# pymc-devs/pymc

Hardware: AMD Instinct MI355X
Metric: effective samples/sec (and leapfrog steps/sec), 10k-param hierarchical logistic regression, one NUTS chain per GPU (higher is better)
Workload: dtype f64

## Files before the change

pymc_amd/csrc/engine.hip:

```cpp
#include <hip/hip_runtime.h>

#include <algorithm>
#include <atomic>
#include <chrono>
#include <cmath>
#include <cstdio>
#include <cstdlib>
#include <cstring>
#include <mutex>
#include <thread>
#include <utility>
#include <ctime>
#include <string>
#include <vector>

#include "kernels.h"
#include "small_kernel.h"
#include "mixture_kernel.h"
#include "loglik_kernel.h"
#include "predictive_kernel.h"
#include "nuts_mi355.h"
#include "pcg64_stream.h"
#include "advi.h"

// ... 53 lines not shown
  int cap = 0, used = 0;
  int64_t ring_full = 0;
  void reset() { side = 0; n = 0; cap = 0; used = 0; }
  template <class F>
  void begin(int d, int dir, int last, F dir_of) {
    cap = 0; used = 0;
    for (int e = d + 1; e <= last; ++e)
      if (dir_of(e) == -dir) { cap = std::min(1 << std::min(e, 30), ring); break; }
  }
  int leaf(int dir, int* slot, int* k) {
    if (n > 0 && side == dir) { *slot = (int)(head % (unsigned)ring); *k = used++; ++head; --n; return EP_REPLAY; }
    if (cap > 0 && n < cap) { side = -dir; *k = n; *slot = (int)((head + (unsigned)n) % (unsigned)ring); ++n; return EP_PAIRED; }
    if (cap > 0 && n >= ring) ++ring_full;
    *slot = -1; *k = -1;
    return EP_PLAIN;
  }
};
extern "C" int64_t nuts_edge_pair_plan(const int32_t* dirs, int32_t n_dirs, int32_t n_doublings, int32_t spec, int32_t max_depth,
                                       int32_t ring, int32_t* out, int64_t out_cap) {
  if (!dirs || !out || n_doublings < 0 || n_doublings > n_dirs || n_doublings > 20 || ring < 1) { g_err = "nuts_edge_pair_plan: bad argument"; return -1; }
  EdgePlan ep;
  ep.ring = ring;
  int64_t n = 0;
  const int last = std::min(std::min(spec, max_depth - 1), n_dirs - 1);
  for (int d = 0; d < n_doublings; ++d) {
    ep.begin(d, dirs[d], last, [&](int e) { return (int)dirs[e]; });
    for (int j = 0; j < (1 << d); ++j, ++n) {
      int slot, k;
      const int kind = ep.leaf(dirs[d], &slot, &k);
      if (n >= out_cap) { g_err = "nuts_edge_pair_plan: output too small"; return -1; }
      int32_t* o = out + 5 * n;
      o[0] = d; o[1] = j; o[2] = kind; o[3] = slot; o[4] = k;
    }
  }
  return n;
}

#define PROF_RUN_MIN 16
#define SMALL_MAX_ELEMS 16384
#define SMALL_MAX_N 1024

struct nuts_model {
  ModelDev md{};
  hipStream_t stream = nullptr;
  std::vector<void*> owned;
  double* q_dev = nullptr;
  double* g_dev = nullptr;
  double* lp_dev = nullptr;
  double* host_pin = nullptr;
  std::vector<nuts_data_ref> data_refs;
  int64_t data_epoch = 0;
  double* set_pin = nullptr; int64_t set_pin_len = 0; hipEvent_t set_ev = nullptr;
  int rows_grid = 0, mvn_grid = 0, ept = 1;
  bool has_prog = false;
  int rows_rpl = 2, rows_alternate = 1, rows_flip = 0, rows_occ = 4;
  int vector_one_xcd = 0;
  int ga_struct_ok = 0;
  int ga_par = 0;
  int64_t dom_units = 0;
  int explicit_pre = 0;
  int64_t alg_bytes = 0;
  bool profile = false;
  std::vector<hipEvent_t> ev;
  std::vector<int32_t> ev_units;
  int run_open = 0;
  int64_t runs_seen = 0;
  size_t ev_used = 0;
  int64_t dom_launches = 0;
  int sample_every = 1;
  hipStream_t own_stream = nullptr;
  struct nuts_group* group = nullptr;
  bool g_active = false;
  int gslot = 0;
  int n_chains = 0;
  int64_t pool_extra = 0;
  int64_t orphan_elems = 0, factor_elems = 0;
  double rows_pack_s = 0.0;
  int64_t rows_xt_len = 0, rows_y_len = 0;
  int ep_ok = 0, ep_par = 0;
  double *ep_ring = nullptr, *ep_part = nullptr, *ep_bpart = nullptr, *ep_def_loc = nullptr;
  int64_t ep_ring_bytes = 0, ep_shadows = 0, ep_replays = 0;
  int64_t ep_dropped = 0;
  int64_t ep_ring_full = 0;
  int ep_turns = 0;
  struct EpLaunch {
    int kind = EP_PLAIN, slot = 0, sj = 0, sfold = 0, first = 0;
    EvalIO sio{}; ArenaDev sA{};
  } ep_launch;
  std::vector<LinDev> lins_host;
  std::vector<nuts_factor> fac_host;
  double *ll_q = nullptr, *ll_stage = nullptr, *ll_par = nullptr, *ll_sc = nullptr, *ll_lfact = nullptr;
  int32_t* ll_dead = nullptr;
  int64_t ll_stage_n = 0, ll_par_n = 0;
  int n_waic = 0;

  template <typename T>
  T* keep(T* p) {
    owned.push_back((void*)p);
    return p;
  }
};

extern "C" int nuts_device_count(void) {
  int n = 0;
  if (hipGetDeviceCount(&n) != hipSuccess) return 0;
  return n;
}
extern "C" int nuts_set_device(int device) {
  HIPCHK(hipSetDevice(device));
  return NUTS_OK;
}
extern "C" const char* nuts_last_error(void) { return g_err.c_str(); }

#define GRP_MAXC MFM_MAXC
struct nuts_group {
  std::mutex mu;
  hipStream_t stream = nullptr;
  nuts_model* member[GRP_MAXC] = {};
  int n = 0;
  int nactive = 0, npend = 0;
  std::atomic<unsigned> gen{0};
  MvaLeafArgs pend[GRP_MAXC];
  int64_t launches[GRP_MAXC + 1] = {};
  int cap = MVM_MAXC;
  ModelDev* md_dev = nullptr;
  const nuts_model* md_of = nullptr;
  double* dpack = nullptr;
  MfmChainConst* konst_dev = nullptr;
  MfmChainConst konst_host[GRP_MAXC] = {};
  bool konst_set[GRP_MAXC] = {};
  int kind = 0;
  GaLeafArgs gpend[GAL_MAXC];
  int rows_flip = 0;
  GalConst* gal_konst_dev = nullptr;
  GalConst gal_konst_host[GAL_MAXC] = {};
  bool gal_konst_set[GAL_MAXC] = {};
  int rows_lds = 1;
};
static_assert(GAM_MAXNC == MVM_MAXC && GAL_MAXC == GAM_MAXC && GAL_MAXC <= GRP_MAXC, "group sizes");

static nuts_model* group_base(nuts_group* g) {
  for (int i = 0; i < GRP_MAXC; ++i) if (g->member[i]) return g->member[i];
  return nullptr;
}

template <typename Leaf, int N>
static void group_order(const Leaf* pend, int nc, int (&order)[N]) {
  for (int a = 0; a < N; ++a) order[a] = a;
  for (int a = 1; a < nc; ++a)
    for (int b = a; b > 0 && pend[order[b]].slot < pend[order[b - 1]].slot; --b) std::swap(order[b], order[b - 1]);
}

static void group_submitted(nuts_group* g, int nc) {
  g->launches[nc]++;
  g->npend = 0;
  g->gen.fetch_add(1, std::memory_order_release);
}

static GalConst gal_const(const GaLeafArgs& L) {
  GalConst k{};
  k.A = L.A; k.A.uniforms = nullptr; k.A.log_uniforms = nullptr; k.Emax = L.Emax; k.st = L.st;
  k.ga_part = L.ga_part; k.ga_bpart = L.ga_bpart; k.ga_ticket = L.ga_ticket; k.def_loc = L.def_loc; k.max_depth = L.max_depth; k.slot = L.slot;
  return k;
}

static void group_flush_rows_locked(nuts_group* g);
// ... 1602 lines not shown
extern "C" int nuts_model_set_data(nuts_model* m, int32_t data_id, const double* values, int64_t n) {
  if (!m || !values) { g_err = "null argument"; return NUTS_E_ARG; }
  if (data_id < 0 || data_id >= (int)m->data_refs.size()) { g_err = "nuts_model_set_data: no such data vector"; return NUTS_E_ARG; }
  const nuts_data_ref& r = m->data_refs[data_id];
  if (n != r.size) { g_err = "nuts_model_set_data: the length of a data vector cannot change"; return NUTS_E_ARG; }
  HIPCHK(hipStreamSynchronize(m->stream));
  HIPCHK(hipMemcpy(const_cast<double*>(m->md.pool) + r.offset, values, (size_t)n * sizeof(double), hipMemcpyHostToDevice));
  m->data_epoch++;
  return NUTS_OK;
}

extern "C" int nuts_model_set_data_many(nuts_model* m, int32_t count, const int32_t* data_ids, const double* values, const int64_t* lens) {
  if (!m || count < 0 || (count > 0 && (!data_ids || !values || !lens))) { g_err = "null argument"; return NUTS_E_ARG; }
  int64_t total = 0;
  for (int i = 0; i < count; ++i) {
    if (data_ids[i] < 0 || data_ids[i] >= (int)m->data_refs.size()) { g_err = "nuts_model_set_data_many: no such data vector"; return NUTS_E_ARG; }
    if (lens[i] != m->data_refs[data_ids[i]].size) { g_err = "nuts_model_set_data_many: the length of a data vector cannot change"; return NUTS_E_ARG; }
    total += lens[i];
  }
  if (total == 0) return NUTS_OK;
  if (m->set_pin_len < total) {
    if (m->set_ev) HIPCHK(hipEventSynchronize(m->set_ev));
    if (m->set_pin) hipHostFree(m->set_pin);
    m->set_pin = nullptr; m->set_pin_len = 0;
    HIPCHK(hipHostMalloc((void**)&m->set_pin, (size_t)total * sizeof(double), hipHostMallocDefault));
    m->set_pin_len = total;
  }
  if (!m->set_ev) HIPCHK(hipEventCreateWithFlags(&m->set_ev, hipEventDisableTiming));
  else HIPCHK(hipEventSynchronize(m->set_ev));
  std::memcpy(m->set_pin, values, (size_t)total * sizeof(double));
  int64_t at = 0;
  for (int i = 0; i < count;) {
    const int64_t off0 = m->data_refs[data_ids[i]].offset;
    int64_t run = lens[i];
    int j = i + 1;
    while (j < count && m->data_refs[data_ids[j]].offset == off0 + run) { run += lens[j]; ++j; }
    if (run > 0)
      HIPCHK(hipMemcpyAsync(const_cast<double*>(m->md.pool) + off0, m->set_pin + at, (size_t)run * sizeof(double), hipMemcpyHostToDevice, m->stream));
    at += run;
    i = j;
  }
  HIPCHK(hipEventRecord(m->set_ev, m->stream));
  m->data_epoch++;
  return NUTS_OK;
}

static void group_remove_model(struct nuts_group* g, nuts_model* m);
extern "C" void nuts_model_destroy(nuts_model* m) {
  if (!m) return;
  if (m->stream) hipStreamSynchronize(m->stream);
  if (m->set_ev) hipEventDestroy(m->set_ev);
  if (m->set_pin) hipHostFree(m->set_pin);
  if (m->group) group_remove_model(m->group, m);
  for (void* p : m->owned) if (p) hipFree(p);
  for (void* p : {(void*)m->ll_q, (void*)m->ll_stage, (void*)m->ll_par, (void*)m->ll_sc, (void*)m->ll_dead, (void*)m->ll_lfact}) if (p) hipFree(p);
  for (auto e : m->ev) hipEventDestroy(e);
  if (m->host_pin) hipHostFree(m->host_pin);
  if (m->own_stream) hipStreamDestroy(m->own_stream);
  delete m;
}

extern "C" int nuts_model_debug_ticks(nuts_model* m, int64_t* out) {
  if (!m || !out) return NUTS_E_ARG;
  HIPCHK(hipStreamSynchronize(m->stream));
  HIPCHK(hipMemcpy(out, m->md.ticks, 64 * sizeof(long long), hipMemcpyDeviceToHost));
  return NUTS_OK;
}

extern "C" int32_t nuts_model_ndim(const nuts_model* m) { return m ? m->md.n : -1; }
extern "C" int nuts_model_get_scalar(const nuts_model* m, const char* name, double* out) {
  if (!m || !name || !out) return NUTS_E_ARG;
  const std::string k(name);
  if (k == "rows_group_aligned") *out = m->md.lg.ga;
  else if (k == "rows_group_block") *out = m->md.lg.ga_gpw;
  else if (k == "rows_packed") *out = m->md.lg.ga ? m->md.lg.ga_pack : 0;
  else if (k == "rows_pack_build_s") *out = m->rows_pack_s;
  else if (k == "edge_pair") *out = m->ep_ok;
  else if (k == "edge_pair_ring_bytes") *out = (double)m->ep_ring_bytes;
  else if (k == "edge_pair_shadows") *out = (double)m->ep_shadows;
  else if (k == "edge_pair_replays") *out = (double)m->ep_replays;
  else if (k == "edge_pair_turns") *out = m->ep_turns;
  else if (k == "edge_pair_dropped") *out = (double)m->ep_dropped;
  else if (k == "edge_pair_ring_full") *out = (double)m->ep_ring_full;
  else if (k == "rows_aux_workgroups") *out = m->md.lg.ga ? m->md.lg.ga_naux : 0;
  else if (k == "mixture_workgroups") *out = m->md.has_mix ? m->md.mix.nwg : 0;
  else if (k == "glm_workgroups") *out = m->md.has_glm ? m->md.glm.nwg : 0;
  else if (k == "glm_row_stride") *out = m->md.has_glm ? m->md.glm.xstride : 0;
  else if (k == "glm_layout_width") *out = m->md.has_glm ? m->md.glm.Ppad : 0;
  else if (k == "mvn_row_aligned") *out = m->md.has_mvn ? m->md.mv.aligned : 0;
  else if (k == "loglik_batch") *out = LL_B;
  else if (k == "loglik_stage_bytes") *out = (double)(m->ll_stage_n * LL_B * (int64_t)sizeof(double));
  else if (k == "rows_waves") *out = m->md.lg.ga ? m->md.lg.ga_w : m->md.lg.n_waves;
  else if (k == "lean") *out = m->md.lean_ok;
  else if (k == "chain_group_kind") {
    const RowsDev& lg = m->md.lg;
    const bool is_mvn = m->md.has_mvn && (m->md.mv.aligned == 4 || m->md.mv.aligned == 8 || m->md.mv.aligned == 16);
    const bool is_rows = m->md.has_logit && !m->md.has_mvn && lg.ga && lg.ga_naux == 0 && lg.D == 8 && m->ga_struct_ok == 1;
    *out = is_mvn ? 1.0 : (is_rows ? (lg.ga_gpw > 0 ? 3.0 : 2.0) : 0.0);
  }
  else if (k == "chain_group_wide_ok") *out = (m->md.has_mvn && m->md.mv.aligned > 0 && m->md.mv.k % 16 == 0) ? 1.0 : 0.0;
  else if (k == "chain_group_wide_rows") *out = 8.0;
  else if (k == "single_workgroup_ok") *out = (m->md.n <= SMALL_MAX_N && m->ept == 1 && !m->md.has_logit && !m->md.has_mvn && !m->md.has_mix && !m->md.has_glm && m->md.n_lins == 0 && m->factor_elems <= SMALL_MAX_ELEMS) ? 1.0 : 0.0;
  else { g_err = "unknown model scalar " + k; return NUTS_E_ARG; }
  return NUTS_OK;
}
extern "C" int64_t nuts_model_algorithmic_bytes(const nuts_model* m) { return m ? m->alg_bytes : 0; }

extern "C" int nuts_model_logp_grad(nuts_model* m, const double* q, double* logp, double* grad) {
  if (!m || !q || !logp) { g_err = "null argument"; return NUTS_E_ARG; }
  const int n = m->md.n;
  std::memcpy(m->host_pin, q, n * sizeof(double));
  HIPCHK(hipMemcpyAsync(m->q_dev, m->host_pin, n * sizeof(double), hipMemcpyHostToDevice, m->stream));
  m->md.fdead_mode = 1;
  model_enqueue_plain(m, m->q_dev, m->g_dev, m->lp_dev);
  m->md.fdead_mode = 0;
  HIPCHK(hipMemcpyAsync(m->host_pin + n, m->g_dev, n * sizeof(double), hipMemcpyDeviceToHost, m->stream));
  HIPCHK(hipMemcpyAsync(m->host_pin + 2 * n, m->lp_dev, sizeof(double), hipMemcpyDeviceToHost, m->stream));
  HIPCHK(hipStreamSynchronize(m->stream));
  HIPCHK(hipGetLastError());
  *logp = m->host_pin[2 * n];
  if (m->md.n_factors > 0 && !std::isfinite(*logp)) {
    std::vector<int32_t> fd(m->md.n_factors);
    HIPCHK(hipMemcpy(fd.data(), m->md.fdead, fd.size() * sizeof(int32_t), hipMemcpyDeviceToHost));
    bool any = false;
    for (int32_t v : fd) any = any || v != 0;
    if (any) {
      if (grad) {
        m->md.fdead_mode = 2;
        model_enqueue_plain(m, m->q_dev, m->g_dev, m->lp_dev);
        m->md.fdead_mode = 0;
        HIPCHK(hipMemcpyAsync(m->host_pin + n, m->g_dev, n * sizeof(double), hipMemcpyDeviceToHost, m->stream));
      }
      HIPCHK(hipMemsetAsync(m->md.fdead, 0, fd.size() * sizeof(int32_t), m->stream));
      HIPCHK(hipStreamSynchronize(m->stream));
      HIPCHK(hipGetLastError());
    }
  }
  if (grad) std::memcpy(grad, m->host_pin + n, n * sizeof(double));
  return NUTS_OK;
}

static int64_t ll_size(nuts_model* m, int kind, int index) {
  const ModelDev& md = m->md;
  switch (kind) {
    case NUTS_LL_FACTOR:
      if (index < 0 || index >= md.n_factors) { g_err = "log-likelihood: the index is not a factor of the model"; return -1; }
      if (m->fac_host[index].dist == NUTS_D_DERIVED) { g_err = "log-likelihood: a derived vector has no log-density of its own"; return -1; }
      return m->fac_host[index].size;
    case NUTS_LL_LOGIT_ROWS: if (md.has_logit) return md.lg.N; break;
    case NUTS_LL_MIXTURE:
      if (md.has_mix && md.mix.assign) {
        g_err = "log-likelihood: the conditional mixture's likelihood depends on assignments another step method rewrites per draw";
        return -1;
      }
      if (md.has_mix) return md.mix.N;
      break;
    case NUTS_LL_GLM: if (md.has_glm) return md.glm.N; break;
    default: g_err = "log-likelihood: unknown kind"; return -1;
  }
  g_err = "log-likelihood: the model has no such node";
  return -1;
}

static int ll_check(nuts_model* m, int kind, int index, int64_t* N) {
  if (!m) { g_err = "null argument"; return NUTS_E_ARG; }
  if (m->group) { g_err = "log-likelihood: the model is a member of a chain group (its stream is the group's); remove the chain first"; return NUTS_E_ARG; }
// ... 589 lines not shown
    log_step = mu - hbar * std::sqrt((double)count) / gamma;
    const double mk = std::pow((double)count, -k);
    log_bar = mk * log_step + (1 - mk) * log_bar;
    count += 1;
  }
};

struct StateHeader {
  int64_t magic, n;
  DualAvg da;
  int64_t iter_count, divergences, n_samples, adaptation_window;
  int32_t tune, fg_is_a, pad0, pad1;
  double fg_count, bg_count;
  int64_t fa_previous_update;
  double fa_fg_n, fa_bg_n;
};

#define DOM_RING 4
struct nuts_chain {
  nuts_model* m = nullptr;
  nuts_chain_config cfg{};
  int n = 0;
  ArenaDev A{};
  std::vector<void*> owned;
  double *var = nullptr, *stds = nullptr, *inv_stds = nullptr;
  double *dense_C = nullptr, *dense_W = nullptr;
  int dense = 0, mv_grid = 0;
  int host_pot = 0, cb_err = 0;
  nuts_velocity_fn hp_velocity = nullptr;
  nuts_energy_fn hp_energy = nullptr;
  nuts_velocity_energy_fn hp_velocity_energy = nullptr;
  void* hp_user = nullptr;
  std::vector<double> hp_p, hp_v;
  double* kin_user_dev = nullptr;
  int full_adapt = 0, fa_mfma = 1;
  double *fa_L = nullptr, *fa_Lw = nullptr, *fa_fg_mean = nullptr, *fa_fg_raw = nullptr, *fa_bg_mean = nullptr, *fa_bg_raw = nullptr;
  double *fa_scratch = nullptr, *fa_rhs = nullptr;
  int *fa_fail = nullptr;
  double fa_fg_n = 0, fa_bg_n = 0;
  int64_t fa_previous_update = 0;
  std::vector<double> fa_initial_cov;
  double *wa_mean = nullptr, *wa_m2 = nullptr, *wb_mean = nullptr, *wb_m2 = nullptr;
  bool fg_is_a = true;
  double fg_count = 0, bg_count = 0;
  std::vector<double> initial_mean, initial_diag;
  int64_t n_samples = 0, adaptation_window = 101;
  bool window_switched = false;
  DualAvg da{};
  bool tune = true;
  int64_t iter_count = 0, divergences = 0;
  double step_size = 0;
  double* stage_dev = nullptr;
  double* stage_host = nullptr;
  double* out_dev = nullptr;
  double* out_dev2 = nullptr;
  bool small = false;
  int small_lds_slots = 0;
  int small_one_wave = 1;
  int group_wide = 0;
  double* out_host = nullptr;
  HostStatus* st_dev = nullptr;
  HostStatus* st_host = nullptr;
  int seq = 0;
  std::vector<double> div_source, div_dest;
  bool cache_ok = false;
  std::vector<double> last_q;
  double last_logp = 0.0;
  DrawOut* do_dev = nullptr;
  DrawOut* do_host = nullptr;
  DrawOutMapped* dom_host = nullptr;
  DrawOutMapped* dom_dev = nullptr;
  unsigned dom_seq = 0;
  double* kin_part = nullptr;
  int64_t cache_epoch = -1;
  int fold_ctl = 1;
  CtlJob pend{}; bool pend_valid = false;
  bool defer_last_ctl = false; int xfold = 1;
  int next_dir = 0; bool pre_done = false; int xpre = 1;
  bool edge_pair = false;
  ArenaDev shA{};
  EdgePlan ep;
  int spec_max = 10, last_depth = 0;
  int pipe_draws = 1;
  int logs_done = 0, logs_total = 0;
  double* many_in_host = nullptr; double* many_in_dev = nullptr; char* many_out_host = nullptr; char* many_out_dev = nullptr;
  size_t many_in_cap = 0, many_out_cap = 0;
  double t_begin = 0, t_loop = 0, t_wait = 0, t_finish = 0, t_post = 0;
  double tm_pre = 0, tm_start = 0, tm_tree = 0, tm_record = 0, tm_host = 0, tm_post = 0;
  int64_t tm_draws = 0, tm_batches = 0;
  int64_t leapfrogs = 0;
  int n_uni_cap = 0;
  template <typename T>
  T* keep(T* p) { owned.push_back((void*)p); return p; }
};

extern "C" void nuts_chain_config_default(nuts_chain_config* c) {
  std::memset(c, 0, sizeof(*c));
  c->step_scale = 0.25; c->Emax = 1000; c->target_accept = 0.8; c->gamma = 0.05; c->k = 0.75; c->t0 = 10;
  c->adapt_step_size = 1; c->max_treedepth = 10; c->early_max_treedepth = 8;
  c->potential = NUTS_POT_DIAG_ADAPT; c->initial_weight = 0; c->adaptation_window = 101; c->discard_window = 50;
  c->exp_alpha = 0.02; c->exp_stop_adaptation = INFINITY; c->exp_use_grads = 0;
  c->adaptation_window_multiplier = 1; c->early_update = 0;
}

static void fa_factor(nuts_chain* c, const double* raw, double denom) {
  const int n = c->n;
  hipStream_t s = c->m->stream;
  const dim3 g2((n + 255) / 256, n);
  hipLaunchKernelGGL(k_fa_cov, g2, dim3(256), 0, s, n, raw, denom, c->dense_C, c->fa_Lw, c->fa_fail);
  const int nb = (n + FA_NB - 1) / FA_NB;
  for (int k = 0; k < nb; ++k) {
    hipLaunchKernelGGL(k_chol_panel, dim3(nb - k), dim3(256), 0, s, n, c->fa_Lw, k, c->fa_fail);
    const int m = nb - k - 1;
    if (m > 0) hipLaunchKernelGGL(k_chol_update, dim3(m * (m + 1) / 2), dim3(256), 0, s, n, c->fa_Lw, k, nb, c->fa_mfma);
  }
  hipLaunchKernelGGL(k_fa_commit, dim3(1024), dim3(256), 0, s, (int64_t)n * n, c->fa_Lw, c->fa_L, c->fa_fail, c->fa_fail + 1);
}
static void fa_random(nuts_chain* c, const double* z_dev, double* p_out) {
  const int n = c->n;
  hipStream_t s = c->m->stream;
  hipMemcpyAsync(c->fa_rhs, z_dev, n * sizeof(double), hipMemcpyDeviceToDevice, s);
  const int nb = (n + FA_NB - 1) / FA_NB;
  for (int b = nb - 1; b >= 0; --b)
    hipLaunchKernelGGL(k_trsv_block, dim3(std::max(1, (b * FA_NB + 255) / 256)), dim3(256), 0, s, n, c->fa_L, c->fa_rhs, p_out, b);
}
static int fa_reset(nuts_chain* c) {
  const int n = c->n;
  const size_t nn = (size_t)n * n;
  const double w = c->cfg.initial_weight;
  std::vector<double> raw(nn);
  for (size_t e = 0; e < nn; ++e) raw[e] = c->fa_initial_cov[e] * w;
  HIPCHK(hipMemcpy(c->fa_fg_raw, raw.data(), nn * sizeof(double), hipMemcpyHostToDevice));
  HIPCHK(hipMemcpy(c->fa_fg_mean, c->initial_mean.data(), n * sizeof(double), hipMemcpyHostToDevice));
  HIPCHK(hipMemset(c->fa_bg_raw, 0, nn * sizeof(double)));
  HIPCHK(hipMemset(c->fa_bg_mean, 0, n * sizeof(double)));
  HIPCHK(hipMemset(c->fa_fail, 0, 2 * sizeof(int)));
  c->fa_fg_n = w; c->fa_bg_n = 0; c->fa_previous_update = 0;
  c->adaptation_window = c->cfg.adaptation_window;
  HIPCHK(hipMemcpy(c->fa_Lw, c->fa_initial_cov.data(), nn * sizeof(double), hipMemcpyHostToDevice));
  {
    hipStream_t s = c->m->stream;
    HIPCHK(hipMemcpyAsync(c->fa_bg_raw, c->fa_Lw, nn * sizeof(double), hipMemcpyDeviceToDevice, s));
    fa_factor(c, c->fa_bg_raw, 1.0);
    HIPCHK(hipMemsetAsync(c->fa_bg_raw, 0, nn * sizeof(double), s));
    HIPCHK(hipStreamSynchronize(s));
  }
  int fail[2] = {0, 0};
  HIPCHK(hipMemcpy(fail, c->fa_fail, sizeof(fail), hipMemcpyDeviceToHost));
  if (fail[0]) { g_err = "the initial covariance of QuadPotentialFullAdapt is not positive definite"; return NUTS_E_LINALG; }
  return NUTS_OK;
}
static int fa_update(nuts_chain* c, const double* x_dev) {
  if (!c->tune) return NUTS_OK;
  const int n = c->n;
  hipStream_t s = c->m->stream;
  const int64_t delta = c->n_samples - c->fa_previous_update;
  c->fa_fg_n += 1; c->fa_bg_n += 1;
  hipLaunchKernelGGL(k_fa_diffs, dim3((n + 255) / 256), dim3(256), 0, s, n, x_dev, c->fa_fg_mean, c->fa_bg_mean, c->fa_fg_n, c->fa_bg_n, c->fa_scratch);
  hipLaunchKernelGGL(k_fa_rank1, dim3((n + 255) / 256, n), dim3(256), 0, s, n, c->fa_scratch, c->fa_fg_raw, c->fa_bg_raw);
  if ((delta + 1) % c->cfg.fa_update_window == 0) fa_factor(c, c->fa_fg_raw, c->fa_fg_n - 1.0);
  if (delta >= c->adaptation_window) {
    std::swap(c->fa_fg_raw, c->fa_bg_raw); std::swap(c->fa_fg_mean, c->fa_bg_mean);
    c->fa_fg_n = c->fa_bg_n; c->fa_bg_n = 0;
    HIPCHK(hipMemsetAsync(c->fa_bg_raw, 0, (size_t)n * n * sizeof(double), s));
    HIPCHK(hipMemsetAsync(c->fa_bg_mean, 0, n * sizeof(double), s));
    c->fa_previous_update = c->n_samples;
// ... 34 lines not shown
  if (cfg->potential < NUTS_POT_DIAG_ADAPT || cfg->potential > NUTS_POT_HOST) { g_err = "unknown potential kind"; return nullptr;
  }
  if (cfg->potential == NUTS_POT_FULL && (!cfg->dense_cov || !cfg->dense_rand)) { g_err = "dense potential needs dense_cov and dense_rand"; return nullptr; }
  if (cfg->potential == NUTS_POT_FULL_ADAPT && !cfg->dense_cov) { g_err = "NUTS_POT_FULL_ADAPT needs dense_cov (the initial covariance)"; return nullptr; }
  if (cfg->max_treedepth < 1 || cfg->max_treedepth > MAX_LEVELS - 1) { g_err = "max_treedepth out of range (1..11)"; return nullptr; }
  if ((cfg->potential == NUTS_POT_FULL || cfg->potential == NUTS_POT_FULL_ADAPT || cfg->potential == NUTS_POT_HOST) && m->md.lg.ga) {
    g_err = "a dense mass matrix needs the span-partitioned row pass: create the model with NUTS_ROWS_NO_GROUP_ALIGNED";
    return nullptr;
  }
  auto* c = new nuts_chain();
  c->m = m; c->cfg = *cfg; c->n = m->md.n;
  m->n_chains++;
  const int n = c->n;
  c->initial_mean.assign(n, 0.0);
  c->initial_diag.assign(n, 1.0);
  if (cfg->initial_mean) c->initial_mean.assign(cfg->initial_mean, cfg->initial_mean + n);
  if (cfg->initial_diag) c->initial_diag.assign(cfg->initial_diag, cfg->initial_diag + n);
  else if (cfg->potential == NUTS_POT_DIAG_ADAPT) c->cfg.initial_weight = 1;
  c->cfg.initial_mean = nullptr; c->cfg.initial_diag = nullptr;
  c->host_pot = cfg->potential == NUTS_POT_HOST;
  c->dense = cfg->potential == NUTS_POT_FULL || cfg->potential == NUTS_POT_FULL_ADAPT || c->host_pot;
  c->full_adapt = cfg->potential == NUTS_POT_FULL_ADAPT;
  c->fa_mfma = env_int("NUTS_FA_MFMA", 1);
  if (c->cfg.fa_update_window < 1) c->cfg.fa_update_window = 1;
  if (c->dense) c->initial_diag.assign(m->md.n, 1.0);
  c->cfg.dense_cov = nullptr; c->cfg.dense_rand = nullptr;
  c->adaptation_window = cfg->adaptation_window;
  ArenaDev& A = c->A;
  A.n = n;
  const int maxd = std::max(cfg->max_treedepth, cfg->early_max_treedepth);
  A.S = 1 << maxd;
  A.ept = m->ept;
  A.nblk = m->md.nblk;
  const size_t arena = (size_t)A.S * n;
  A.Q = c->keep(dev_alloc<double>(arena)); A.P = c->keep(dev_alloc<double>(arena));
  A.V = c->keep(dev_alloc<double>(arena)); A.G = c->keep(dev_alloc<double>(arena));
  A.E = c->keep(dev_alloc<double>(A.S)); A.LOGP = c->keep(dev_alloc<double>(A.S));
  A.PS = c->keep(dev_alloc<double>((size_t)MAX_LEVELS * n));
  A.PSUM = c->keep(dev_alloc<double>(n));
  c->kin_part = c->keep(dev_alloc<double>((size_t)A.nblk));
  A.ctl = c->keep(dev_alloc<Ctl>(1));
  c->var = c->keep(dev_alloc<double>(n)); c->stds = c->keep(dev_alloc<double>(n)); c->inv_stds = c->keep(dev_alloc<double>(n));
  c->wa_mean = c->keep(dev_alloc<double>(n)); c->wa_m2 = c->keep(dev_alloc<double>(n));
  c->wb_mean = c->keep(dev_alloc<double>(n)); c->wb_m2 = c->keep(dev_alloc<double>(n));
  A.var = c->var; A.inv_stds = c->inv_stds;
  A.ga_ticket = m->md.lg.ga ? m->md.lg.ga_ticket : nullptr; A.ga_nticket = m->md.lg.ga ? 2 * m->md.lg.ga_nblk : 0;
  if (c->full_adapt) {
    const size_t nn = (size_t)n * n;
    c->fa_initial_cov.assign(cfg->dense_cov, cfg->dense_cov + nn);
    c->dense_C = c->keep(dev_alloc<double>(nn));
    c->fa_L = c->keep(dev_alloc<double>(nn)); c->fa_Lw = c->keep(dev_alloc<double>(nn));
    c->fa_fg_raw = c->keep(dev_alloc<double>(nn)); c->fa_bg_raw = c->keep(dev_alloc<double>(nn));
    c->fa_fg_mean = c->keep(dev_alloc<double>(n)); c->fa_bg_mean = c->keep(dev_alloc<double>(n));
    c->fa_scratch = c->keep(dev_alloc<double>(4 * (size_t)n)); c->fa_rhs = c->keep(dev_alloc<double>(n));
    c->fa_fail = c->keep(dev_alloc<int>(2));
    c->mv_grid = (n + (256 / WAVE) - 1) / (256 / WAVE);
  } else if (c->host_pot) {
    c->hp_p.assign(n, 0.0); c->hp_v.assign(n, 0.0);
    c->kin_user_dev = c->keep(dev_alloc<double>(1));
    A.kin_user = c->kin_user_dev;
  } else if (c->dense) {
    c->dense_C = c->keep(dev_upload(cfg->dense_cov, (size_t)n * n));
    c->dense_W = c->keep(dev_upload(cfg->dense_rand, (size_t)n * n));
    c->mv_grid = (n + (256 / WAVE) - 1) / (256 / WAVE);
  }
  c->n_uni_cap = (1 << maxd) + 2 * maxd + 16;
  c->stage_dev = c->keep(dev_alloc<double>(2 * (size_t)n + 2 * (size_t)c->n_uni_cap));
  c->out_dev = c->keep(dev_alloc<double>(2 * (size_t)n));
  c->out_dev2 = c->keep(dev_alloc<double>(2 * (size_t)n + 2));
  c->fold_ctl = env_int("NUTS_FOLD_CTL", 1) != 0 && !(m->md.has_mvn && m->md.mv.winv);
  c->spec_max = env_int("NUTS_SPEC_MAX", 10);
  c->xfold = env_int("NUTS_XFOLD", 1);
  c->edge_pair = m->ep_ok && env_int("NUTS_EDGE_PAIR", 1) != 0 && !c->dense && !c->host_pot && !m->md.has_mvn && !m->explicit_pre &&
                 m->md.lean_ok && c->fold_ctl && c->xfold;
  if (c->edge_pair) {
    c->shA = A;
    c->shA.S = 2;
    c->shA.Q = c->keep(dev_alloc<double>(2 * (size_t)n)); c->shA.P = c->keep(dev_alloc<double>(2 * (size_t)n));
    c->shA.V = c->keep(dev_alloc<double>(2 * (size_t)n)); c->shA.G = c->keep(dev_alloc<double>(2 * (size_t)n));
    if (!c->shA.Q || !c->shA.P || !c->shA.V || !c->shA.G) { (void)hipGetLastError(); c->edge_pair = false; }
    c->ep.ring = std::max(1, std::min(GA_RING_LEAVES, env_int("NUTS_EDGE_PAIR_RING", GA_RING_LEAVES)));
  }
  c->pipe_draws = env_int("NUTS_PIPE_DRAWS", 1) != 0;
  c->xpre = env_int("NUTS_XPRE", 1);
  c->small_lds_slots = env_int("NUTS_SMALL_LDS", 1) == 0 ? -1 : env_int("NUTS_SMALL_LDS_SLOTS", 0);
  c->small_one_wave = env_int("NUTS_SMALL_ONE_WAVE", 1);
  c->group_wide = env_int("NUTS_GROUP_WIDE", 0);
  const bool glm_small = m->md.has_glm && env_int("NUTS_GLM_SMALL", 1) != 0 && m->md.glm.Xt && !m->md.glm.beta_buf && m->md.glm.off_beta >= 0 && m->md.n_derived == 0 && n <= 256;
  c->small = env_int("NUTS_SMALL_KERNEL", 1) != 0 && n <= SMALL_MAX_N && m->ept == 1 && !m->md.has_logit && !m->md.has_mvn && !m->md.has_mix &&
             (!m->md.has_glm || glm_small) &&
             m->md.n_lins == 0 && m->factor_elems <= SMALL_MAX_ELEMS && !c->dense;
  c->do_dev = c->keep(dev_alloc<DrawOut>(1));
  A.uniforms = c->stage_dev + 2 * (size_t)n;
  A.log_uniforms = A.uniforms + c->n_uni_cap;
  for (void* p : c->owned)
    if (!p) { g_err = "device allocation failed (trajectory arena needs 4*2^max_treedepth*n*8 bytes)"; nuts_chain_destroy(c); return nullptr; }
  if (hipHostMalloc((void**)&c->stage_host, (2 * (size_t)n + 2 * (size_t)c->n_uni_cap) * sizeof(double), hipHostMallocDefault) != hipSuccess ||
      hipHostMalloc((void**)&c->out_host, 2 * (size_t)n * sizeof(double), hipHostMallocDefault) != hipSuccess ||
      hipHostMalloc((void**)&c->st_host, sizeof(HostStatus), hipHostMallocMapped) != hipSuccess ||
      hipHostGetDevicePointer((void**)&c->st_dev, c->st_host, 0) != hipSuccess ||
      hipHostMalloc((void**)&c->do_host, sizeof(DrawOut), hipHostMallocDefault) != hipSuccess ||
      hipHostMalloc((void**)&c->dom_host, DOM_RING * sizeof(DrawOutMapped), hipHostMallocMapped) != hipSuccess ||
      hipHostGetDevicePointer((void**)&c->dom_dev, c->dom_host, 0) != hipSuccess) {
    g_err = "pinned host allocation failed"; nuts_chain_destroy(c); return nullptr;
  }
  hipMemset(A.ctl, 0, sizeof(Ctl));
  std::memset(c->st_host, 0, sizeof(HostStatus));
  std::memset(c->dom_host, 0, DOM_RING * sizeof(DrawOutMapped));
  c->step_size = cfg->step_scale / std::pow((double)n, 0.25);
  c->da = DualAvg{c->step_size, cfg->target_accept, cfg->gamma, cfg->k, cfg->t0, 0, 0, 0, 0, 1};
  c->da.reset();
  if (potential_reset(c) != NUTS_OK) { nuts_chain_destroy(c); return nullptr; }
  return c;
}

extern "C" void nuts_chain_destroy(nuts_chain* c) {
  if (!c) return;
  if (c->m) hipStreamSynchronize(c->m->stream);
  if (c->m && c->m->group) group_remove_model(c->m->group, c->m);
  if (c->m) c->m->n_chains--;
  for (void* p : c->owned) if (p) hipFree(p);
  if (c->stage_host) hipHostFree(c->stage_host);
  if (c->out_host) hipHostFree(c->out_host);
  if (c->st_host) hipHostFree(c->st_host);
  if (c->do_host) hipHostFree(c->do_host);
  if (c->dom_host) hipHostFree(c->dom_host);
  if (c->many_in_host) hipHostFree(c->many_in_host);
  if (c->many_out_host) hipHostFree(c->many_out_host);
  if (c->many_in_dev) hipFree(c->many_in_dev);
  if (c->many_out_dev) hipFree(c->many_out_dev);
  delete c;
}

static void group_remove_model(nuts_group* g, nuts_model* m) {
  if (!g || !m || m->group != g) return;
  hipStreamSynchronize(g->stream);
  std::lock_guard<std::mutex> lk(g->mu);
  for (int i = 0; i < GRP_MAXC; ++i)
    if (g->member[i] == m) { g->member[i] = nullptr; g->n--; g->konst_set[i] = false; if (i < GAL_MAXC) g->gal_konst_set[i] = false; }
  if (m->g_active) { g->nactive--; m->g_active = false; }
  m->group = nullptr;
  m->stream = m->own_stream;
}

extern "C" nuts_group* nuts_group_create(void) {
  nuts_group* g = new nuts_group();
  if (hipStreamCreateWithFlags(&g->stream, hipStreamNonBlocking) != hipSuccess) { g_err = "nuts_group_create: no stream"; delete g; return nullptr; }
  return g;
}

extern "C" int nuts_group_add(nuts_group* g, nuts_chain* c) {
  if (!g || !c || !c->m) return NUTS_E_ARG;
  nuts_model* m = c->m;
  const MvnDev& mv = m->md.mv;
  if (m->group) { g_err = "nuts_group_add: the chain's model already belongs to a group"; return NUTS_E_ARG; }
  if (m->n_chains != 1) { g_err = "nuts_group_add: a member model carries exactly one chain (its launch parity and records are the chain's)"; return NUTS_E_ARG; }
  const RowsDev& lg = m->md.lg;
  const bool is_mvn = m->md.has_mvn && (mv.aligned == 4 || mv.aligned == 8);
  const bool is_rows = m->md.has_logit && !m->md.has_mvn && lg.ga && lg.ga_naux == 0 && lg.D == 8 && m->ga_struct_ok == 1;
  const int rows_kind = lg.ga_gpw > 0 ? 3 : 2;
  if (!(is_mvn || is_rows) || c->dense || c->host_pot) {
    g_err = "nuts_group_add: chain groups advance models that are one constant-covariance MvNormal node on the row-aligned pass or the "
            "hierarchical-logit rows on the group-aligned pass (diagonal mass matrix); this chain is neither";
    return NUTS_E_ARG;
  }
  const int rows_lds = g->n == 0 ? env_int("NUTS_ROWS_GROUP_LDS", 1) : g->rows_lds;
// ... 692 lines not shown
  const bool cached0 = start_cached(c, q0);
  double* const h_q = c->many_in_host;
  double* const h_norm = h_q + n;
  double* const h_u = h_norm + (size_t)K * n;
  double* const h_lu = h_u + U;
  std::memcpy(h_q, q0, n * sizeof(double));
  std::memcpy(h_norm, normals, (size_t)K * n * sizeof(double));
  std::memcpy(h_u, uniforms, U * sizeof(double));
  for (size_t i = 0; i < U; ++i) h_lu[i] = std::log(h_u[i]);
  HIPCHK(hipMemcpyAsync(c->many_in_dev, c->many_in_host, in_doubles * sizeof(double), hipMemcpyHostToDevice, s));
  const double* const d_norm = c->many_in_dev + n;
  const double* const d_u = d_norm + (size_t)K * n;
  const double* const d_lu = d_u + U;
  double* const trace_dev = reinterpret_cast<double*>(c->many_out_dev);
  if (!cached0) {
    HIPCHK(hipMemcpyAsync(A.Q, c->many_in_dev, n * sizeof(double), hipMemcpyDeviceToDevice, s));
    model_enqueue_plain(c->m, A.Q, A.G, A.LOGP);
  }
  const double* const save_u = A.uniforms; const double* const save_lu = A.log_uniforms;
  const int save_done = c->logs_done, save_total = c->logs_total;
  c->logs_done = c->logs_total = 1 << 30;
  int done = 0;
  size_t consumed = 0;
  const int fgrid = std::max(1, std::min(256, (n + VEC_THREADS - 1) / VEC_THREADS));
  c->tm_pre += secs(tm0, clk::now()); c->tm_batches++;
  const bool pipe = !c->tune && !c->full_adapt && c->pipe_draws;
  struct Pending {
    bool valid = false; int k = 0; unsigned seq = 0; bool exhausted = false, adapt = false; size_t consumed_after = 0; int cursor = 0;
    double perf_start = 0.0, wall = 0.0, cpu = 0.0;
  } pend;
  auto enqueue_start = [&](int k, const DrawPlan& plan, size_t at, bool from_prev) {
    A.uniforms = d_u + at; A.log_uniforms = d_lu + at;
    return enqueue_draw_start(c, d_norm + (size_t)k * n, false, from_prev, plan.step_size, 0, plan.max_depth, k > 0 ? (const DrawOut*)c->do_dev : nullptr);
  };
  auto complete = [&](const Pending& p, bool* diverged) -> int {
    const auto tb = clk::now();
    DrawOutMapped* slot = c->dom_host + (p.seq % DOM_RING);
    unsigned long long seen = 0;
    int r = wait_seq(c, &slot->seq, 0, p.seq, "k_draw_finish ended without publishing its record", &seen);
    if (r) return r;
    const DrawOut o = slot->o;
    const auto t1 = clk::now();
    c->tm_record += secs(tb, t1);
    if (o.cursor != p.cursor) { g_err = "internal error: the status word and the draw record disagree on the uniforms consumed"; return NUTS_E_HIP; }
    r = finish_draw_host(c, o, p.adapt, p.exhausted, c->out_dev, o.n_proposals + ((p.k == 0 && !cached0) ? 1 : 0), p.perf_start, p.wall, p.cpu,
                         stats + p.k);
    c->tm_host += secs(t1, clk::now()); c->tm_draws++;
    if (r) return r;
    stats[p.k].n_uniforms_consumed = (int32_t)p.consumed_after;
    c->last_logp = o.logp;
    done = p.k + 1;
    *diverged = o.diverging != 0;
    return NUTS_OK;
  };
  bool started = false;
  for (int k = 0; k < K; ++k) {
    const DrawClock dclock;
    const DrawPlan plan = plan_draw(c);
    const size_t need_uni = (size_t)plan.need_uni;
    if (!started) {
      if (U - consumed < need_uni) {
        if (k == 0) { g_err = "not enough uniforms for the worst-case tree"; rc = NUTS_E_ARG; }
        break;
      }
      rc = enqueue_start(k, plan, consumed, k > 0 || cached0);
      if (rc) break;
    }
    started = false;
    unsigned flags = 0;
    bool exhausted = true;
    int cursor = 0;
    const auto ta = clk::now();
    c->tm_start += secs(dclock.t0, ta);
    rc = run_tree(c, h_u + consumed, plan.step_size, plan.max_depth, &flags, &exhausted, &cursor);
    const auto tb = clk::now();
    c->tm_tree += secs(ta, tb);
    if (rc) break;
    if (flags & ST_BAD_ENERGY) {
      if (pend.valid) { bool dv = false; rc = complete(pend, &dv); pend.valid = false; if (rc) break; }
      rc = bad_initial_energy(c);
      break;
    }
    const unsigned seq = ++c->dom_seq;
    hipLaunchKernelGGL(k_draw_finish, dim3(fgrid), dim3(VEC_THREADS), 0, s, A, c->out_dev, c->out_dev + n, c->do_dev, trace_dev + (size_t)k * n,
                       c->dom_dev + (seq % DOM_RING), seq);
    const size_t consumed_after = consumed + (size_t)cursor;
    if (pipe && !(flags & ST_DIVERGING) && k + 1 < K && U - consumed_after >= need_uni) {
      rc = enqueue_start(k + 1, plan, consumed_after, true);
      if (rc) break;
      started = true;
    }
    Pending cur;
    cur.valid = true; cur.k = k; cur.seq = seq; cur.exhausted = exhausted; cur.adapt = plan.adapt; cur.consumed_after = consumed_after; cur.cursor = cursor;
    cur.perf_start = dclock.perf_start(); cur.wall = dclock.wall(); cur.cpu = dclock.cpu();
    bool diverged = false;
    if (pend.valid) { rc = complete(pend, &diverged); pend.valid = false; if (rc) break; }
    if (started) pend = cur;
    else { rc = complete(cur, &diverged); if (rc) break; }
    consumed = consumed_after;
    if (diverged) break;
  }
  if (pend.valid) {
    bool dv = false;
    const int r2 = complete(pend, &dv);
    pend.valid = false;
    if (!rc) rc = r2;
  }
  A.uniforms = save_u; A.log_uniforms = save_lu;
  c->logs_done = save_done; c->logs_total = save_total;
  *n_done = done;
  const auto tm1 = clk::now();
  struct PostTimer { nuts_chain* c; clk::time_point t; ~PostTimer() { c->tm_post += secs(t, clk::now()); } } post_timer{c, tm1};
  if (done > 0) {
    HIPCHK(hipMemcpyAsync(c->many_out_host, c->many_out_dev, (size_t)done * n * sizeof(double), hipMemcpyDeviceToHost, s));
    HIPCHK(hipStreamSynchronize(s));
    HIPCHK(hipGetLastError());
    const double* trace_host = reinterpret_cast<const double*>(c->many_out_host);
    std::memcpy(q_out, trace_host, (size_t)done * n * sizeof(double));
    commit_start_cache(c, trace_host + (size_t)(done - 1) * n, c->last_logp);
  } else {
    hipStreamSynchronize(s);
  }
  if (rc && done > 0 && rc != NUTS_E_BAD_ENERGY) return rc;
  return done > 0 ? NUTS_OK : (rc ? rc : NUTS_E_ARG);
}

extern "C" int nuts_chain_draw_many(nuts_chain* c, const double* q0, const double* normals, const double* uniforms,
                                    int32_t n_uniforms, int32_t K, double* q_out, nuts_draw_stats* stats, int32_t* n_done) {
  if (!c || !q0 || !normals || !uniforms || !q_out || !stats || !n_done || K <= 0) { g_err = "null argument"; return NUTS_E_ARG; }
  if (c->host_pot) { g_err = "nuts_chain_draw_many: a host potential is consulted between draws (random, update): one nuts_chain_draw per transition"; return NUTS_E_ARG; }
  if (!c->small) return draw_many_general(c, q0, normals, uniforms, n_uniforms, K, q_out, stats, n_done);
  if (c->tune) { g_err = "nuts_chain_draw_many: the chain is still tuning (the single-launch batch has no adaptation between its draws)"; return NUTS_E_ARG; }
  const DrawClock dclock;
  const int n = c->n;
  hipStream_t s = c->m->stream;
  ArenaDev& A = c->A;
  const DrawPlan plan = plan_draw(c);
  if (n_uniforms < plan.need_uni) { g_err = "not enough uniforms for the worst-case tree"; return NUTS_E_ARG; }
  const size_t in_doubles = (size_t)n + (size_t)K * n + (size_t)n_uniforms;
  const size_t trace_bytes = (size_t)K * n * sizeof(double), outs_bytes = (size_t)K * sizeof(DrawOut);
  const size_t out_bytes = trace_bytes + outs_bytes + 16;
  int rc = ensure_many_staging(c, in_doubles, out_bytes);
  if (rc) return rc;
  const bool cached = start_cached(c, q0);
  std::memcpy(c->many_in_host, q0, n * sizeof(double));
  std::memcpy(c->many_in_host + n, normals, (size_t)K * n * sizeof(double));
  std::memcpy(c->many_in_host + n + (size_t)K * n, uniforms, (size_t)n_uniforms * sizeof(double));
  HIPCHK(hipMemcpyAsync(c->many_in_dev, c->many_in_host, in_doubles * sizeof(double), hipMemcpyHostToDevice, s));
  if (!cached) HIPCHK(hipMemcpyAsync(A.Q, c->many_in_dev, n * sizeof(double), hipMemcpyDeviceToDevice, s));
  ArenaDev Am = A;
  Am.uniforms = c->many_in_dev + n + (size_t)K * n;
  SmallDrawArgs a = small_draw_args(c, cached, plan);
  a.normals = c->many_in_dev + n;
  a.n_draws = K; a.n_uniforms = n_uniforms;
  a.trace_q = reinterpret_cast<double*>(c->many_out_dev);
  a.out = reinterpret_cast<DrawOut*>(c->many_out_dev + trace_bytes);
  a.n_done = reinterpret_cast<int*>(c->many_out_dev + trace_bytes + outs_bytes);
  launch_small(c, Am, a);
  std::swap(c->out_dev, c->out_dev2);
  HIPCHK(hipMemcpyAsync(c->many_out_host, c->many_out_dev, out_bytes, hipMemcpyDeviceToHost, s));
  HIPCHK(hipStreamSynchronize(s));
  HIPCHK(hipGetLastError());
  const double* trace_host = reinterpret_cast<const double*>(c->many_out_host);
  const DrawOut* outs = reinterpret_cast<const DrawOut*>(c->many_out_host + trace_bytes);
  const int done = *reinterpret_cast<const int*>(c->many_out_host + trace_bytes + outs_bytes);
  *n_done = done;
  if (done <= 0 || done > K) { g_err = "nuts_chain_draw_many: the device reported an impossible draw count"; return NUTS_E_HIP; }
  if (outs[done - 1].bad_energy) return bad_initial_energy(c);
  const double wall = dclock.wall() / done, cpu = dclock.cpu() / done;
  for (int i = 0; i < done; ++i) {
    const DrawOut& o = outs[i];
    c->divergences += o.diverging != 0;
    c->iter_count += 1;
// ... 844 lines not shown
```

pymc_amd/csrc/kernels.h:

```cpp
#pragma once
#include "model_dev.h"
#include "rows_kernel.h"

#define MAX_LEVELS 12
#define NDOT (1 + 6 * (MAX_LEVELS + 1))
#define DOT_TOP (1 + 6 * MAX_LEVELS)
#define VEC_THREADS 256
#define PART_STRIDE (PART_DOT + NDOT)

#define ROWS_BLOCK 256

#define MODE_PLAIN 0
#define MODE_TREE 1
#define MODE_SIMPLE 2

struct Ctl {
  double E0;
  double log_size, log_accept_sum, max_energy_change;
  double div_dE;
  int n_proposals, depth, left, right, proposal, cursor;
  int aborted, turning, diverging, bad_energy;
  int dir, edge;
  double eps;
  double eps_abs;
// ... 1522 lines not shown
    const int i = base + e * VEC_THREADS + threadIdx.x;
    if (i < A.n) {
      double p, v;
      if (dense) { p = A.P[i]; v = A.V[i]; }
      else {
        p = p_exact ? p_exact[i] : normals[i] * A.inv_stds[i];
        v = A.var[i] * p;
        A.P[i] = p; A.V[i] = v;
      }
      A.PSUM[i] = p;
      if (q_src) { A.Q[i] = q_src[i]; A.G[i] = g_src[i]; }
      kin = fma(p, v, kin);
    }
  }
  const double tot = block_sum<false>(kin, sm);
  if (threadIdx.x == 0) kin_part[blockIdx.x] = tot;
}

struct DrawOut {
  double energy, logp, E0, log_accept_sum, max_energy_change, div_dE;
  int depth, n_proposals, proposal, cursor, turning, diverging, bad_energy, div_t;
};

__global__ void k_draw_ctl_start(ArenaDev A, const double* __restrict__ kin_part, double step_size, int dir_forced, int max_depth,
                                 HostStatus* st, int use_cached_logp, double cached_logp, const DrawOut* prev) {
  if (threadIdx.x == 0) {
    double s = 0.0;
    for (int b = 0; b < A.nblk; ++b) s += kin_part[b];
    Ctl* c = A.ctl;
    if (use_cached_logp) A.LOGP[0] = prev ? prev->logp : cached_logp;
    const double logp = A.LOGP[0];
    const double E = (A.kin_user ? *A.kin_user : 0.5 * s) - logp;
    A.E[0] = E;
    c->E0 = E;
    c->log_size = 0.0;
    c->log_accept_sum = -INFINITY;
    c->max_energy_change = 0.0;
    c->div_dE = 0.0;
    c->n_proposals = 0; c->depth = 0; c->left = 0; c->right = 0; c->proposal = 0; c->cursor = 0;
    c->turning = 0; c->diverging = 0;
    c->bad_energy = !isfinite(E);
    c->aborted = c->bad_energy;
    c->eps_abs = step_size;
    c->n_leaves_total = 0;
    c->dir = 1; c->edge = 0; c->eps = step_size;
    if (dir_forced != 0) { c->dir = dir_forced; c->eps = dir_forced > 0 ? step_size : -step_size; }
    else if (!c->aborted && max_depth > 0) ctl_next_direction(c, A.uniforms);
    if (st) publish_fields(c, st);
  }
}


struct DrawOutMapped { DrawOut o; unsigned long long seq; };

__global__ __launch_bounds__(VEC_THREADS) void k_draw_finish(ArenaDev A, double* __restrict__ q_out,
                                                             double* __restrict__ g_out, DrawOut* out,
                                                             double* __restrict__ trace_q, DrawOutMapped* mapped, unsigned seq) {
  const Ctl* c = A.ctl;
  const int prop = c->proposal;
  const int64_t po = slot_off(A, prop);
  if (blockIdx.x == 0) for (int t = threadIdx.x; t < A.ga_nticket; t += blockDim.x) A.ga_ticket[t] = 0u;
  for (int i = blockIdx.x * blockDim.x + threadIdx.x; i < A.n; i += gridDim.x * blockDim.x) {
    const double qi = A.Q[po + i];
    q_out[i] = qi;
    g_out[i] = A.G[po + i];
    if (trace_q) trace_q[i] = qi;
  }
  if (blockIdx.x == 0 && threadIdx.x == 0) {
    const int ps = prop & (A.S - 1);
    DrawOut o;
    o.energy = A.E[ps]; o.logp = A.LOGP[ps]; o.E0 = c->E0;
    o.log_accept_sum = c->log_accept_sum; o.max_energy_change = c->max_energy_change; o.div_dE = c->div_dE;
    o.depth = c->depth; o.n_proposals = c->n_proposals; o.proposal = prop; o.cursor = c->cursor;
    o.turning = c->turning; o.diverging = c->diverging; o.bad_energy = c->bad_energy; o.div_t = c->div_t;
    *out = o;
    if (mapped) {
      mapped->o = o;
      __threadfence_system();
      __hip_atomic_store(&mapped->seq, (unsigned long long)seq, __ATOMIC_RELEASE, __HIP_MEMORY_SCOPE_SYSTEM);
    }
  }
}

__global__ __launch_bounds__(VEC_THREADS) void k_potential_update(int n, const double* __restrict__ x,
                                                                  double* fg_mean, double* fg_m2, double fg_count_new,
                                                                  double* bg_mean, double* bg_m2, double bg_count_new,
                                                                  double* var, double* stds, double* inv_stds, int flags) {
  for (int i = blockIdx.x * blockDim.x + threadIdx.x; i < n; i += gridDim.x * blockDim.x) {
    double m2 = fg_m2[i];
    if (flags & 1) {
      const double xi = x[i];
      double mean = fg_mean[i];
      double od = xi - mean;
      mean += od / fg_count_new;
      m2 += od * (xi - mean);
      fg_mean[i] = mean; fg_m2[i] = m2;
      double bm = bg_mean[i], b2 = bg_m2[i];
      od = xi - bm;
      bm += od / bg_count_new;
      b2 += od * (xi - bm);
      bg_mean[i] = bm; bg_m2[i] = b2;
    }
    if (flags & 2) {
      double v = m2 / fg_count_new;
      v = fmin(fmax(v, 1e-12), 1e12);
      if (isnan(m2 / fg_count_new)) v = m2 / fg_count_new;
      const double s = sqrt(v);
      var[i] = v; stds[i] = s; inv_stds[i] = 1.0 / s;
    }
  }
}

__global__ __launch_bounds__(VEC_THREADS) void k_potential_update_exp(int n, const double* __restrict__ x, const double* __restrict__ g,
                                                                      double* ms, double* vs, double* mg, double* vg, double alpha,
                                                                      double one_m_alpha, int use_grads, double* var, double* stds,
                                                                      double* inv_stds, int flags) {
  for (int i = blockIdx.x * blockDim.x + threadIdx.x; i < n; i += gridDim.x * blockDim.x) {
    if (flags & 1) {
      ms[i] = x[i]; vs[i] = 0.0;
      if (use_grads) { mg[i] = g[i]; vg[i] = 0.0; }
    }
    if (flags & 2) {
      {
        const double delta = __dsub_rn(x[i], ms[i]);
        ms[i] = __dadd_rn(ms[i], __dmul_rn(alpha, delta));
        vs[i] = __dmul_rn(one_m_alpha, __dadd_rn(vs[i], __dmul_rn(alpha, __dmul_rn(delta, delta))));
      }
      if (use_grads) {
        const double delta = __dsub_rn(g[i], mg[i]);
        mg[i] = __dadd_rn(mg[i], __dmul_rn(alpha, delta));
        vg[i] = __dmul_rn(one_m_alpha, __dadd_rn(vg[i], __dmul_rn(alpha, __dmul_rn(delta, delta))));
      }
    }
    if (flags & 4) {
      double v;
      if (use_grads) v = __dsqrt_rn(__ddiv_rn(vs[i], vg[i]));
      else { v = vs[i]; v = fmin(fmax(v, 1e-12), 1e12); if (isnan(vs[i])) v = vs[i]; }
      const double sd = __dsqrt_rn(v);
      var[i] = v; stds[i] = sd; inv_stds[i] = __ddiv_rn(1.0, sd);
    }
  }
}

#include "rows_ga_kernel.h"
#include "rows_gb_kernel.h"
#include "dense_adapt.h"
#include "glm_kernel.h"
#include "mvn_multi_kernel.h"
#include "mvn_mfma_kernel.h"
#include "rows_ga_multi_kernel.h"
#include "rows_gal_kernel.h"
#include "rows_gb_multi_kernel.h"
#include "lin_kernel.h"
```

Measured before the change: 20190.

## Fuse draw finish with next trajectory start into one kernel

Adds k_draw_turn, a kernel that writes out the accepted draw, then reinitializes the arena for the next NUTS trajectory: it copies position and gradient, samples momentum, computes kinetic energy via a last-block ticket reduction, and resets the control block. It replaces the separate k_draw_finish launch plus enqueue_start sequence on the pipelined path, removing launches and a dependency gap between draws. In exchange it duplicates start logic in the kernel and relies on a grid-wide ticket counter, so it could diverge from enqueue_start semantics, for example adaptation or potential updates done between draws.

```diff
diff --git a/pymc_amd/csrc/engine.hip b/pymc_amd/csrc/engine.hip
--- a/pymc_amd/csrc/engine.hip
+++ b/pymc_amd/csrc/engine.hip
@@ -159,6 +159,7 @@
   int64_t ep_ring_bytes = 0, ep_shadows = 0, ep_replays = 0;
   int64_t ep_dropped = 0;
   int64_t ep_ring_full = 0;
+  int64_t draw_turns_fused = 0;
   int ep_turns = 0;
   struct EpLaunch {
     int kind = EP_PLAIN, slot = 0, sj = 0, sfold = 0, first = 0;
@@ -1927,6 +1928,9 @@
   else if (k == "edge_pair_turns") *out = m->ep_turns;
   else if (k == "edge_pair_dropped") *out = (double)m->ep_dropped;
   else if (k == "edge_pair_ring_full") *out = (double)m->ep_ring_full;
+  else if (k == "draw_turns_fused") *out = (double)m->draw_turns_fused;
+  else if (k == "vec_workgroups") *out = m->md.nblk;
+  else if (k == "vec_elems_per_thread") *out = m->ept;
   else if (k == "rows_aux_workgroups") *out = m->md.lg.ga ? m->md.lg.ga_naux : 0;
   else if (k == "mixture_workgroups") *out = m->md.has_mix ? m->md.mix.nwg : 0;
   else if (k == "glm_workgroups") *out = m->md.has_glm ? m->md.glm.nwg : 0;
@@ -2682,6 +2686,8 @@
   EdgePlan ep;
   int spec_max = 10, last_depth = 0;
   int pipe_draws = 1;
+  bool draw_turn = false;
+  unsigned* turn_ticket = nullptr;
   int logs_done = 0, logs_total = 0;
   double* many_in_host = nullptr; double* many_in_dev = nullptr; char* many_out_host = nullptr; char* many_out_dev = nullptr;
   size_t many_in_cap = 0, many_out_cap = 0;
@@ -2882,6 +2888,9 @@
     c->ep.ring = std::max(1, std::min(GA_RING_LEAVES, env_int("NUTS_EDGE_PAIR_RING", GA_RING_LEAVES)));
   }
   c->pipe_draws = env_int("NUTS_PIPE_DRAWS", 1) != 0;
+  c->draw_turn = env_int("NUTS_DRAW_TURN", 1) != 0 && !c->dense && !c->host_pot;
+  c->turn_ticket = c->keep(dev_alloc<unsigned>(1));
+  if (c->turn_ticket) hipMemset(c->turn_ticket, 0, sizeof(unsigned));
   c->xpre = env_int("NUTS_XPRE", 1);
   c->small_lds_slots = env_int("NUTS_SMALL_LDS", 1) == 0 ? -1 : env_int("NUTS_SMALL_LDS_SLOTS", 0);
   c->small_one_wave = env_int("NUTS_SMALL_ONE_WAVE", 1);
@@ -3740,13 +3749,23 @@
       break;
     }
     const unsigned seq = ++c->dom_seq;
-    hipLaunchKernelGGL(k_draw_finish, dim3(fgrid), dim3(VEC_THREADS), 0, s, A, c->out_dev, c->out_dev + n, c->do_dev, trace_dev + (size_t)k * n,
-                       c->dom_dev + (seq % DOM_RING), seq);
     const size_t consumed_after = consumed + (size_t)cursor;
-    if (pipe && !(flags & ST_DIVERGING) && k + 1 < K && U - consumed_after >= need_uni) {
-      rc = enqueue_start(k + 1, plan, consumed_after, true);
-      if (rc) break;
+    const bool start_next = pipe && !(flags & ST_DIVERGING) && k + 1 < K && U - consumed_after >= need_uni;
+    if (start_next && c->draw_turn) {
+      A.uniforms = d_u + consumed_after; A.log_uniforms = d_lu + consumed_after;
+      hipLaunchKernelGGL(k_draw_turn, dim3(A.nblk), dim3(VEC_THREADS), 0, s, A, c->out_dev, c->out_dev + n, c->do_dev, trace_dev + (size_t)k * n,
+                         c->dom_dev + (seq % DOM_RING), seq, d_norm + (size_t)(k + 1) * n, c->kin_part, c->turn_ticket, plan.step_size,
+                         plan.max_depth, c->st_dev);
+      c->m->draw_turns_fused++;
       started = true;
+    } else {
+      hipLaunchKernelGGL(k_draw_finish, dim3(fgrid), dim3(VEC_THREADS), 0, s, A, c->out_dev, c->out_dev + n, c->do_dev, trace_dev + (size_t)k * n,
+                         c->dom_dev + (seq % DOM_RING), seq);
+      if (start_next) {
+        rc = enqueue_start(k + 1, plan, consumed_after, true);
+        if (rc) break;
+        started = true;
+      }
     }
     Pending cur;
     cur.valid = true; cur.k = k; cur.seq = seq; cur.exhausted = exhausted; cur.adapt = plan.adapt; cur.consumed_after = consumed_after; cur.cursor = cursor;
diff --git a/pymc_amd/csrc/kernels.h b/pymc_amd/csrc/kernels.h
--- a/pymc_amd/csrc/kernels.h
+++ b/pymc_amd/csrc/kernels.h
@@ -1628,6 +1628,82 @@
   }
 }
 
+__global__ __launch_bounds__(VEC_THREADS) void k_draw_turn(ArenaDev A, double* __restrict__ q_out, double* __restrict__ g_out, DrawOut* out,
+                                                           double* __restrict__ trace_q, DrawOutMapped* mapped, unsigned seq,
+                                                           const double* __restrict__ normals, double* kin_part, unsigned* ticket,
+                                                           double step_size, int max_depth, HostStatus* st) {
+  __shared__ double sm[VEC_THREADS];
+  __shared__ int s_last;
+  Ctl* c = A.ctl;
+  const int tid = threadIdx.x;
+  const int prop = __hip_atomic_load(&c->proposal, __ATOMIC_RELAXED, __HIP_MEMORY_SCOPE_WAVEFRONT);
+  const int64_t po = slot_off(A, prop);
+  if (blockIdx.x == 0) for (int t = tid; t < A.ga_nticket; t += VEC_THREADS) A.ga_ticket[t] = 0u;
+  double kin = 0.0;
+  const int base = blockIdx.x * VEC_THREADS * A.ept;
+  for (int e = 0; e < A.ept; ++e) {
+    const int i = base + e * VEC_THREADS + tid;
+    if (i < A.n) {
+      const double qi = A.Q[po + i], gi = A.G[po + i];
+      q_out[i] = qi; g_out[i] = gi;
+      if (trace_q) trace_q[i] = qi;
+      A.Q[i] = qi; A.G[i] = gi;
+      const double p = normals[i] * A.inv_stds[i];
+      const double v = A.var[i] * p;
+      A.P[i] = p; A.V[i] = v;
+      A.PSUM[i] = p;
+      kin = fma(p, v, kin);
+    }
+  }
+  const double tot = block_sum<false>(kin, sm);
+  if (tid == 0) {
+    st_agent(kin_part + blockIdx.x, tot);
+    asm volatile("s_waitcnt vmcnt(0)" ::: "memory");
+    const unsigned old = __hip_atomic_fetch_add(ticket, 1u, __ATOMIC_RELAXED, __HIP_MEMORY_SCOPE_AGENT);
+    const int is_last = old + 1u == gridDim.x;
+    if (is_last) __hip_atomic_store(ticket, 0u, __ATOMIC_RELAXED, __HIP_MEMORY_SCOPE_AGENT);
+    s_last = is_last;
+  }
+  __syncthreads();
+  if (!s_last) return;
+  double s = 0.0;
+  for (int b0 = 0; b0 < A.nblk; b0 += VEC_THREADS) {
+    if (b0 + tid < A.nblk) sm[tid] = ld_agent(kin_part + b0 + tid);
+    __syncthreads();
+    if (tid == 0) for (int b = 0; b < min(VEC_THREADS, A.nblk - b0); ++b) s += sm[b];
+    __syncthreads();
+  }
+  if (tid != 0) return;
+  const int ps = prop & (A.S - 1);
+  DrawOut o;
+  o.energy = A.E[ps]; o.logp = A.LOGP[ps]; o.E0 = c->E0;
+  o.log_accept_sum = c->log_accept_sum; o.max_energy_change = c->max_energy_change; o.div_dE = c->div_dE;
+  o.depth = c->depth; o.n_proposals = c->n_proposals; o.proposal = prop; o.cursor = c->cursor;
+  o.turning = c->turning; o.diverging = c->diverging; o.bad_energy = c->bad_energy; o.div_t = c->div_t;
+  *out = o;
+  mapped->o = o;
+  __threadfence_system();
+  __hip_atomic_store(&mapped->seq, (unsigned long long)seq, __ATOMIC_RELEASE, __HIP_MEMORY_SCOPE_SYSTEM);
+  A.LOGP[0] = o.logp;
+  const double logp = o.logp;
+  const double E = 0.5 * s - logp;
+  A.E[0] = E;
+  c->E0 = E;
+  c->log_size = 0.0;
+  c->log_accept_sum = -INFINITY;
+  c->max_energy_change = 0.0;
+  c->div_dE = 0.0;
+  c->n_proposals = 0; c->depth = 0; c->left = 0; c->right = 0; c->proposal = 0; c->cursor = 0;
+  c->turning = 0; c->diverging = 0;
+  c->bad_energy = !isfinite(E);
+  c->aborted = c->bad_energy;
+  c->eps_abs = step_size;
+  c->n_leaves_total = 0;
+  c->dir = 1; c->edge = 0; c->eps = step_size;
+  if (!c->aborted && max_depth > 0) ctl_next_direction(c, A.uniforms);
+  if (st) publish_fields(c, st);
+}
+
 __global__ __launch_bounds__(VEC_THREADS) void k_potential_update(int n, const double* __restrict__ x,
                                                                   double* fg_mean, double* fg_m2, double fg_count_new,
                                                                   double* bg_mean, double* bg_m2, double bg_count_new,
```

New measurement: 20280 (median of 4 runs). No clear change (+0.5%).
